# ZikangXiong/mobrob

Hardware: AMD Instinct MI355X
Metric: env-steps/sec (whole node), doggo PPO (higher is better)
Workload: dtype f32

## Files before the change

include/mobrob_ppo.h:

```cpp
#ifndef MOBROB_PPO_H
#define MOBROB_PPO_H

#include <stddef.h>
#include <stdint.h>

#ifdef __cplusplus
extern "C" {
#endif

#define MOBROB_PPO_ABI_VERSION 3
enum { MOBROB_ACT_TANH = 0, MOBROB_ACT_RELU = 1, MOBROB_ACT_ELU = 2, MOBROB_ACT_LEAKY_RELU = 3, MOBROB_ACT_SIGMOID = 4,
       MOBROB_ACT_SOFTPLUS = 5, MOBROB_ACT_SOFTSIGN = 6, MOBROB_ACT_HARDTANH = 7, MOBROB_ACT_RELU6 = 8, MOBROB_ACT_SILU = 9,
       MOBROB_ACT_GELU = 10, MOBROB_ACT_MISH = 11, MOBROB_ACT_COUNT = 12 };

enum {
  MOBROB_OK = 0,
  MOBROB_ERR_INVALID = -1,
  MOBROB_ERR_HIP = -2,
  MOBROB_ERR_STATE = -3,
  MOBROB_ERR_NO_DEVICE = -4
};

typedef struct mobrob_ppo_engine mobrob_ppo_engine_t;

// ... 439 lines not shown
  MOBROB_BUF_RETURNS = 7,
  MOBROB_BUF_PARAMS = 8,
  MOBROB_BUF_GRADS = 9,
  MOBROB_BUF_ADVSTAT = 10,
  MOBROB_BUF_LAST_VALUES = 11,
  MOBROB_BUF_LAST_DONES = 12,
  MOBROB_BUF_CLIPPED_ACTIONS = 13,
  MOBROB_BUF_EPISODE_START_STATE = 14,
  MOBROB_BUF_TERMINAL_OBS = 15,
  MOBROB_BUF_TERMINAL_VALUES = 16,
  MOBROB_BUF_TRUNCATED = 17,
  MOBROB_BUF_ENV_STATE = 18,
  MOBROB_BUF_GRAD_EXCHANGE = 19,
  MOBROB_BUF_SDE_NOISE = 20,
  MOBROB_BUF_COUNT = 21
};
int mobrob_ppo_buffer_info(mobrob_ppo_engine_t* e, int32_t which, void** ptr_dev, size_t* bytes);
int mobrob_ppo_read_buffer(mobrob_ppo_engine_t* e, int32_t which, void* host_out, size_t bytes);
int mobrob_ppo_write_buffer(mobrob_ppo_engine_t* e, int32_t which, const void* host_in, size_t bytes);
int mobrob_ppo_mark_rollout_ready(mobrob_ppo_engine_t* e);

int mobrob_ppo_x3_mode(const mobrob_ppo_engine_t* e);
int mobrob_ppo_update_mode(const mobrob_ppo_engine_t* e);

int mobrob_ppo_explained_variance(mobrob_ppo_engine_t* e, double* out);

int mobrob_ppo_compute_gae(mobrob_ppo_engine_t* e);

int mobrob_ppo_feistel_permutation(mobrob_ppo_engine_t* e, int64_t n, uint64_t key, int64_t* out);

enum {
  MOBROB_K_ACT = 0,
  MOBROB_K_GAE = 1,
  MOBROB_K_TRAIN_GRAD = 2,
  MOBROB_K_APPLY = 3,
  MOBROB_K_ENV = 4,
  MOBROB_K_GRAD_REDUCE = 5,
  MOBROB_K_ALLREDUCE = 6,
  MOBROB_K_COUNT = 7
};
int mobrob_ppo_profile_enable(mobrob_ppo_engine_t* e, int32_t on);
int mobrob_ppo_profile_read(mobrob_ppo_engine_t* e, double* ms , int64_t* calls );

#ifdef __cplusplus
}
#endif
// ... 2 lines not shown
```

mobrob_amd/_lib.py:

```python
from __future__ import annotations

import ctypes as C
import os

_HERE = os.path.dirname(os.path.abspath(__file__))
LIB_PATH = os.environ.get("MOBROB_PPO_LIB") or os.path.join(_HERE, "libmobrob_ppo.so")
ABI_VERSION = 3

OK, ERR_INVALID, ERR_HIP, ERR_STATE, ERR_NO_DEVICE = 0, -1, -2, -3, -4

BUF = dict(obs=0, actions=1, rewards=2, episode_starts=3, values=4, log_probs=5, advantages=6, returns=7,
           params=8, grads=9, advstat=10, last_values=11, last_dones=12, clipped_actions=13, episode_start_state=14,
           terminal_obs=15, terminal_values=16, truncated=17, env_state=18, grad_exchange=19, sde_noise=20)
HYPER = dict(learning_rate=0, clip_range=1, clip_range_vf=2, target_kl=3, ent_coef=4, vf_coef=5, epoch_kernel=6)
KERNEL_IDS = dict(act=0, gae=1, train_grad=2, apply=3, env=4, grad_reduce=5, allreduce=6)


class Config(C.Structure):
    _fields_ = [
        ("abi_version", C.c_int32), ("obs_dim", C.c_int32), ("act_dim", C.c_int32),
        ("pi_hidden", C.c_int32 * 2), ("vf_hidden", C.c_int32 * 2),
        ("n_envs", C.c_int32), ("n_steps", C.c_int32), ("batch_size", C.c_int32), ("n_epochs", C.c_int32),
        ("gamma", C.c_double), ("gae_lambda", C.c_double), ("clip_range", C.c_double), ("ent_coef", C.c_double),
        ("vf_coef", C.c_double), ("max_grad_norm", C.c_double), ("learning_rate", C.c_double),
# ... 202 lines not shown
                                                   C.POINTER(C.c_int32), C.POINTER(C.c_int32), C.POINTER(C.c_int32), C.POINTER(C.c_int32),
                                                   C.POINTER(C.c_int32), C.POINTER(C.c_int32), C.POINTER(C.c_uint16), C.c_int32, _U8,
                                                   C.POINTER(C.c_int32), C.POINTER(C.c_int32), C.POINTER(C.c_int32), C.POINTER(C.c_int32),
                                                   C.POINTER(C.c_int32), C.POINTER(C.c_int32)]),
    "mobrob_ppo_plan_grid_team_smooth": (C.c_int, [_P, C.POINTER(PlanSpec), C.POINTER(WallsC), C.POINTER(HazardFramesC), C.POINTER(PlanTime),
                                                   C.c_int32, C.c_int32, C.c_int32, C.c_int32, _F, _F, _F, C.POINTER(C.c_int32),
                                                   C.POINTER(C.c_int32), C.POINTER(C.c_int32), C.POINTER(C.c_int32), C.POINTER(C.c_int32),
                                                   C.POINTER(C.c_int32), C.POINTER(C.c_int32), C.POINTER(C.c_int32), C.POINTER(C.c_int32),
                                                   C.POINTER(C.c_uint16), C.c_int32, C.POINTER(C.c_int32), C.c_int32, _U8,
                                                   C.POINTER(C.c_int32), C.POINTER(C.c_int32)]),
    "mobrob_ppo_plan_assign": (C.c_int, [_P, C.POINTER(PlanSpec), C.POINTER(WallsC), C.POINTER(HazardsC), C.POINTER(HazardFramesC),
                                         C.POINTER(PlanTime), C.c_int32, C.c_int32, _F, _F, C.POINTER(C.c_int32), _F, C.POINTER(C.c_int32),
                                         _I64, C.POINTER(C.c_int32), _I64, _I64, C.POINTER(C.c_int32), C.POINTER(C.c_int32)]),
    "mobrob_ppo_sde_reset_noise": (C.c_int, [_P]),
    "mobrob_ppo_sde_set_noise": (C.c_int, [_P, _F]),
    "mobrob_ppo_buffer_info": (C.c_int, [_P, C.c_int32, C.POINTER(_P), C.POINTER(C.c_size_t)]),
    "mobrob_ppo_read_buffer": (C.c_int, [_P, C.c_int32, _P, C.c_size_t]),
    "mobrob_ppo_write_buffer": (C.c_int, [_P, C.c_int32, _P, C.c_size_t]),
    "mobrob_ppo_mark_rollout_ready": (C.c_int, [_P]),
    "mobrob_ppo_compute_gae": (C.c_int, [_P]),
    "mobrob_ppo_explained_variance": (C.c_int, [_P, C.POINTER(C.c_double)]),
    "mobrob_ppo_x3_mode": (C.c_int, [_P]),
    "mobrob_ppo_update_mode": (C.c_int, [_P]),
    "mobrob_ppo_feistel_permutation": (C.c_int, [_P, C.c_int64, C.c_uint64, _I64]),
    "mobrob_ppo_profile_enable": (C.c_int, [_P, C.c_int32]),
    "mobrob_ppo_profile_read": (C.c_int, [_P, C.POINTER(C.c_double), _I64]),
}

ALLREDUCE_FN = C.CFUNCTYPE(C.c_int, C.c_void_p, C.c_void_p, C.c_size_t, C.c_int32, C.c_void_p)

_lib = None


class EngineError(RuntimeError):
    pass


def load():
    global _lib
    if _lib is not None:
        return _lib
    if not os.path.exists(LIB_PATH):
        raise ImportError(f"{LIB_PATH} not built. Run `python -c 'import __graft_entry__ as g; g.build()'` "
                          "(hipcc --offload-arch=gfx950). mobrob_amd has no CPU fallback.")
    lib = C.CDLL(LIB_PATH)
    for name, (res, args) in SYMBOLS.items():
# ... 16 lines not shown
```

mobrob_amd/csrc/engine.hip:

```cpp
#include <hip/hip_runtime.h>
#include <rccl/rccl.h>
#include <dlfcn.h>

#include <algorithm>
#include <atomic>
#include <thread>
#include <cmath>
#include <cstdarg>
#include <cstdio>
#include <climits>
#include <cstring>
#include <ctime>
#include <cstdlib>
#include <string>
#include <vector>

#ifdef MOBROB_POISON_LDS
namespace mobrob {
__global__ __launch_bounds__(1024) void k_poison_lds() {
  extern __shared__ unsigned poison_words[];
  volatile unsigned* w = poison_words;
  for (int i = threadIdx.x; i < 160 * 256; i += 1024) w[i] = 0xFFFFFFFFu;
}
inline void poison_lds(hipStream_t st) {
// ... 149 lines not shown
  unsigned adv_pass = 0;
  bool epoch_open = false;
  float* stats = nullptr;
  int stats_cap = 0, stats_n = 0;
  int cur_count = 0;
  bool grad_pending = false;
  double clip_vf = -1.0;
  double target_kl = -1.0;
  int last_epochs_started = 0, last_stopped_early = 0, last_steps_applied = 0;
  ncclComm_t comm = nullptr;
  int64_t allreduce_calls = 0, allreduce_bytes = 0;
  struct OneShot {
    char* xbuf = nullptr;
    size_t payload = 0;
    char* peer[kOneShotMaxRanks] = {nullptr};
    int world = 0, rank = -1;
    bool ready = false;
    unsigned long long seq = 0;
    int* error = nullptr;
    long long timeout_ticks = 0;
  } oneshot;
  double* norm_rec_sum = nullptr; int* norm_rec_t = nullptr; int* fold_idx_dev = nullptr;
  int fold_start[kMaxTensors + 1] = {0};
  bool use_norm_records = false;
  bool epoch_kernel_on = true;
  unsigned* epoch_bar = nullptr;
  float* epoch_consts = nullptr;
  int* epoch_idx = nullptr;
  char* epoch_stage = nullptr;
  int* epoch_err_host = nullptr;
  hipEvent_t epoch_ev = nullptr;
  int last_update_mode = 0;
  float* epoch_snap = nullptr;
  int rollout64_tile_max = 256;
  int pair64_min_tiles = 65;
  int split64_max_tiles = 64;
  float *Xg = nullptr, *actg = nullptr, *lpg = nullptr, *advg = nullptr, *retg = nullptr, *oldvg = nullptr;
  float *hp[kMaxHidden] = {nullptr}, *hv[kMaxHidden] = {nullptr}, *mu = nullptr, *vout = nullptr;
  float *dmu = nullptr, *dv = nullptr, *dzp[kMaxHidden] = {nullptr}, *dzv[kMaxHidden] = {nullptr};
  float *pred_obs = nullptr, *pred_act = nullptr;
  int gemm_tiles = 0;
  bool sde = false, sde_hold = false;
  float *sde_E = nullptr, *sde_E1 = nullptr, *sde_lat2 = nullptr, *sde_gsig = nullptr, *sde_graw = nullptr;
  float *sde_S2 = nullptr, *sde_var = nullptr;
  SdeMode sde_mode{1, 0};
  hipStream_t cstream = nullptr;
  hipEvent_t ev_in = nullptr, ev_k = nullptr, ev_store = nullptr;
// ... 403 lines not shown
}
FusedTrainArgs train256_args(const mobrob_ppo_engine* e) {
  const FusedState& f = e->fused;
  FusedTrainArgs a{};
  a.net[0] = f.net[0]; a.net[1] = f.net[1];
  a.obs = e->obs; a.Dp = e->Dp; a.A = e->A; a.rec = f.train_rec; a.RW = train_rec_width(e->A);
  fill_loss_hyper(e, a);
  a.slabs = f.slabs; a.slab_floats = f.slab_floats; a.sums = e->grads + e->P; a.stamps = f.stamps;
  return a;
}
template <class Args>
Args reduce_args(const mobrob_ppo_engine* e) {
  Args s{};
  s.slabs = e->fused.slabs; s.grads = e->grads; s.P = e->P;
  for (int i = 0; i < 14; ++i) s.offs[i] = e->offs[i];
  s.D = e->D; s.A = e->A; s.ent_coef = (float)e->cfg.ent_coef; s.sums = e->grads + e->P;
  s.rec_sum = e->use_norm_records ? e->norm_rec_sum : nullptr; s.rec_t = e->norm_rec_t;
  return s;
}
Slab64ReduceArgs slab64_reduce_args(const mobrob_ppo_engine* e) { return reduce_args<Slab64ReduceArgs>(e); }
SlabReduceArgs slab_reduce_args(const mobrob_ppo_engine* e) {
  SlabReduceArgs s = reduce_args<SlabReduceArgs>(e);
  s.slab_floats = e->fused.slab_floats; s.Dp = e->Dp; s.h16 = e->A <= 16;
  return s;
}
StatsArgs stats_args(const mobrob_ppo_engine* e) {
  StatsArgs st{};
  st.loss_sums = e->grads + e->P; st.log_std = e->params + e->offs[T_LOGSTD]; st.n_act = e->A; st.sde = e->sde;
  st.ent_coef = (float)e->cfg.ent_coef; st.vf_coef = (float)e->cfg.vf_coef;
  return st;
}
int fused_carve_packs(mobrob_ppo_engine* e) {
  FusedState& f = e->fused;
  const int H = f.H;
  const size_t nW1 = (size_t)(H / 32) * (e->Dp / 8) * 256, nW2 = (size_t)(H / 32) * (H / 8) * 256;
  const size_t nW3f = (size_t)(H / 8) * 256, nW3b = (size_t)(H / 32) * 4 * 256;
  const size_t nW3h = (size_t)(H / 16) * 256;
  const size_t per_net = nW1 + 2 * nW2 + nW3f + nW3h + nW3b + 2 * H;
  f.packed_floats = 2 * per_net;
  CHK(dalloc(e, &f.packed, f.packed_floats));
  const int head_bias[2] = {T_AB, T_VB};
  for (int n = 0; n < 2; ++n) {
    float* p = f.packed + n * per_net;
    f.net[n].W1f = reinterpret_cast<const f32x4*>(p); p += nW1;
    f.net[n].W2f = reinterpret_cast<const f32x4*>(p); p += nW2;
    f.net[n].W3f = reinterpret_cast<const f32x4*>(p); p += nW3f;
// ... 43 lines not shown
          unsigned* w1 = nullptr; unsigned* w2 = nullptr; unsigned* w2b = nullptr; float* w3 = nullptr; float* w3b = nullptr;
          CHK(dalloc(e, &w1, (size_t)K1 * 16 * 768));
          CHK(dalloc(e, &w2, (size_t)8 * 16 * 768));
          CHK(dalloc(e, &w2b, (size_t)8 * 16 * 768));
          CHK(dalloc(e, &w3, (size_t)16 * 64 * 4));
          CHK(dalloc(e, &w3b, (size_t)16 * 64 * 4));
          f.net[n].W1c = w1; f.net[n].W2c = w2; f.net[n].W2bc = w2b; f.net[n].W3c = w3; f.net[n].W3bc = w3b;
        }
        f.lds_chain_bytes = chain_lds_bytes(e->Dp);
      }
    }
    CHK(dalloc(e, &f.train_rec, (size_t)e->N * e->T * train_rec_width(e->A)));
    f.lds_bytes = fused_lds_bytes(e->Dp);
    f.lds_act_bytes = fused_lds_act_bytes(e->Dp);
  }
  return dalloc(e, &f.stamps, 32);
}
int build_norm_record_tables(mobrob_ppo_engine* e) {
  const FusedState& f = e->fused;
  const int nb = cdiv(f.slab_floats, 256);
  CHK(dalloc(e, &e->norm_rec_sum, (size_t)2 * nb * kNormRec));
  CHK(dalloc(e, &e->norm_rec_t, (size_t)2 * nb * kNormRec));
  CHK(dalloc(e, &e->fold_idx_dev, (size_t)2 * nb * kNormRec));
  const SlabReduceArgs s256 = slab_reduce_args(e);
  const Slab64ReduceArgs s64 = slab64_reduce_args(e);
  std::vector<std::vector<int>> per_tensor(13);
  for (int net = 0; net < 2; ++net)
    for (int b = 0; b < nb; ++b) {
      std::vector<int> recs;
      for (int w = 0; w < 4; ++w) {
        std::vector<int> wave;
        for (int l = 0; l < 64; ++l) {
          const int p = b * 256 + w * 64 + l;
          const int dst = p < f.slab_floats ? (f.H == 64 ? slab64_to_canonical(s64, net, p) : slab_to_canonical(s256, net, p)) : -1;
          const int t = tensor_of_canonical(e->offs, e->P, dst);
          if (t >= 0 && std::find(wave.begin(), wave.end(), t) == wave.end()) wave.push_back(t);
        }
        for (int t : wave)
          if (recs.empty() || recs.back() != t) recs.push_back(t);
      }
      if ((int)recs.size() > kNormRec) return fail(MOBROB_ERR_INVALID, "norm record table: %zu tensors in one reduction block", recs.size());
      for (size_t k = 0; k < recs.size(); ++k) per_tensor[recs[k]].push_back((net * nb + b) * kNormRec + (int)k);
    }
  std::vector<int> fold;
  for (int t = 0; t < 13; ++t) {
    e->fold_start[t] = (int)fold.size();
    fold.insert(fold.end(), per_tensor[t].begin(), per_tensor[t].end());
  }
  e->fold_start[13] = (int)fold.size();
  if (fold.size() > 1024) return fail(MOBROB_ERR_INVALID, "norm record table too large (%zu)", fold.size());
  if (!e->plan_only)
    HIPC(hipMemcpyAsync(e->fold_idx_dev, fold.data(), fold.size() * sizeof(int), hipMemcpyHostToDevice, e->stream));
  if (!e->plan_only) HIPC(hipStreamSynchronize(e->stream));
  return MOBROB_OK;
}

int fused_init(mobrob_ppo_engine* e) {
  FusedState& f = e->fused;
  f.enabled = e->cfg.fast_kernels && e->cfg.activation == MOBROB_ACT_TANH && e->Lp == 2 && e->Lv == 2 && !e->sde &&
              fused_shape_ok(e->D, e->A, e->H1, e->H2, e->G1, e->G2);
  if (!f.enabled) return MOBROB_OK;
  f.D = e->D; f.Dp = e->Dp; f.A = e->A; f.H = e->H1;
  if ((uint64_t)(e->T + 1) * e->N * e->Dp * 4ull >= (1ull << 32) || (uint64_t)e->T * e->N * e->A * 4ull >= (1ull << 32) ||
      (uint64_t)e->T * e->N * train_rec_width(e->A) * 4ull >= (1ull << 32)) {
    f.enabled = false;
    return MOBROB_OK;
  }
  CHK(fused_carve_packs(e));
  CHK(fused_alloc_buffers(e));
  if (!e->plan_only) HIPC(fused_set_lds_attr(f));
  return build_norm_record_tables(e);
}
// ... 390 lines not shown
  HIPC(hipMemcpyAsync(e->chunks_dev, e->chunk_table.data(), e->chunk_table.size() * sizeof(NormChunk), hipMemcpyHostToDevice, e->stream));
  std::vector<float> ones(e->N, 1.0f);
  HIPC(hipMemcpyAsync(e->prev_dones, ones.data(), (size_t)e->N * 4, hipMemcpyHostToDevice, e->stream));
  HIPC(hipStreamSynchronize(e->stream));
  repack(e);
  if (e->sde) sde_resample(e, 0, e->N, e->draw_counter++, nullptr, true);
  HIPC(hipStreamSynchronize(e->stream));
  return MOBROB_OK;
}

}

extern "C" {

int mobrob_ppo_device_bytes(const mobrob_ppo_config_t* cfg, size_t* bytes) {
  if (!cfg || !bytes) return fail(MOBROB_ERR_INVALID, "null argument");
  CHK(check_cfg(cfg));
  mobrob_ppo_engine plan;
  plan.plan_only = true;
  CHK(engine_dims(&plan, cfg));
  CHK(engine_alloc(&plan));
  *bytes = plan.arena_used;
  return MOBROB_OK;
}

void* mobrob_ppo_device_alloc(int32_t device_id, size_t bytes) {
  void* p = nullptr;
  if (hipSetDevice(device_id) != hipSuccess || hipMalloc(&p, bytes) != hipSuccess) {
    fail(MOBROB_ERR_HIP, "device_alloc(%zu bytes) failed", bytes);
    return nullptr;
  }
  return p;
}
void mobrob_ppo_device_free(void* p) { if (p) (void)hipFree(p); }

int mobrob_ppo_create(const mobrob_ppo_config_t* cfg, mobrob_ppo_engine_t** out) {
  if (!cfg || !out) return fail(MOBROB_ERR_INVALID, "null argument");
  return engine_create(cfg, nullptr, 0, out);
}

int mobrob_ppo_create_in_arena(const mobrob_ppo_config_t* cfg, void* arena, size_t arena_bytes, mobrob_ppo_engine_t** out) {
  if (!cfg || !out || !arena) return fail(MOBROB_ERR_INVALID, "null argument");
  return engine_create(cfg, arena, arena_bytes, out);
}

void mobrob_ppo_destroy(mobrob_ppo_engine_t* e) {
// ... 1024 lines not shown

int mobrob_ppo_minibatch_grad(mobrob_ppo_engine_t* e, int32_t mb) {
  if (!e) return fail(MOBROB_ERR_INVALID, "null engine");
  if (!e->epoch_open) return fail(MOBROB_ERR_STATE, "minibatch_grad before epoch_begin");
  if (mb < 0 || mb >= e->nmb) return fail(MOBROB_ERR_INVALID, "minibatch %d out of range [0,%d)", mb, e->nmb);
  const int start = mb * e->Bl, B = std::min(e->Bl, e->N * e->T - start);
  const float inv_bg = 1.0f / (float)((int64_t)B * e->cfg.world_size);
  e->cur_count = B;
  if (!e->fused.enabled) generic_minibatch_grad(e, mb, start, B, inv_bg);
  else if (e->fused.H == 64) fused64_minibatch_grad(e, mb, start, B, inv_bg);
  else fused_minibatch_grad(e, mb, start, B, inv_bg);
  HIPC(hipGetLastError());
  e->grad_pending = true;
  return MOBROB_OK;
}

namespace {
void fill_adam_pack_args(mobrob_ppo_engine* e, AdamPackArgs& a) {
  a.p = e->params; a.g = e->grads; a.m = e->m; a.v = e->v; a.P = e->P;
  a.chunks = e->chunks_dev; a.partial = e->chunk_partial; a.nchunks = e->nchunks;
  if (e->use_norm_records) {
    a.partial = e->norm_rec_sum; a.fold_idx = e->fold_idx_dev;
    for (int i = 0; i <= kMaxTensors; ++i) a.fold_start[i] = e->fold_start[i];
  }
  a.max_norm = (float)e->cfg.max_grad_norm; a.beta1 = (float)e->cfg.adam_beta1; a.beta2 = (float)e->cfg.adam_beta2;
  a.eps = (float)e->cfg.adam_eps;
  for (int i = 0; i <= kMaxTensors; ++i) a.offs[i] = e->offs[i];
  a.ntens = e->ntens; a.two_by_two = e->Lp == 2 && e->Lv == 2; a.id_pw1 = T_PW1; a.id_vw1 = T_VW1; a.id_aw = T_AW; a.id_vw = T_VW; a.HL = e->HL; a.GL = e->GL;
  a.D = e->D; a.Dp = e->Dp; a.A = e->A; a.Ap = e->Ap; a.H1 = e->H1; a.H2 = e->H2; a.G1 = e->G1; a.G2 = e->G2;
  a.pW1p = e->pW1p; a.vW1p = e->vW1p; a.aWp = e->aWp; a.vWp = e->vWp;
  for (int n = 0; n < 2; ++n) {
    const bool on = e->fused.enabled;
    a.fW1f[n] = on ? (float*)e->fused.net[n].W1f : nullptr;
    a.fW2f[n] = on ? (float*)e->fused.net[n].W2f : nullptr;
    a.fW3f[n] = on ? (float*)e->fused.net[n].W3f : nullptr;
    const bool ch = on && e->fused.train_chain;
    a.fW2b[n] = on && !ch ? (float*)e->fused.net[n].W2b : nullptr;
    a.fW3b[n] = on && !ch ? (float*)e->fused.net[n].W3b : nullptr;
    a.fW3h[n] = (on && (n == 1 || e->fused.A <= 16)) ? (float*)e->fused.net[n].W3h : nullptr;
    a.fb1s[n] = on ? (float*)e->fused.net[n].b1s : nullptr;
    a.fb2s[n] = on ? (float*)e->fused.net[n].b2s : nullptr;
    const bool x3 = on && e->fused.train_x3;
    a.xW1[n] = x3 ? reinterpret_cast<unsigned short*>(const_cast<unsigned*>(e->fused.net[n].W1x)) : nullptr;
    a.xW2[n] = x3 ? reinterpret_cast<unsigned short*>(const_cast<unsigned*>(e->fused.net[n].W2x)) : nullptr;
    a.xW2b[n] = x3 && !ch ? reinterpret_cast<unsigned short*>(const_cast<unsigned*>(e->fused.net[n].W2bx)) : nullptr;
    a.cW1[n] = ch ? reinterpret_cast<unsigned short*>(const_cast<unsigned*>(e->fused.net[n].W1c)) : nullptr;
    a.cW2[n] = ch ? reinterpret_cast<unsigned short*>(const_cast<unsigned*>(e->fused.net[n].W2c)) : nullptr;
// ... 12 lines not shown
  return {(float)(e->cfg.learning_rate / bc1), (float)std::sqrt(bc2)};
}
int next_stats_row(mobrob_ppo_engine* e) {
  if (e->stats_n >= e->stats_cap) e->stats_n = 0;
  return e->stats_n++;
}
StatsArgs apply_norms(mobrob_ppo_engine* e) {
  StatsArgs st = stats_args(e);
  st.stats_row = e->stats + (size_t)next_stats_row(e) * 8;
  st.inv_bg = 1.0f / (float)((int64_t)e->cur_count * e->cfg.world_size);
  if (!e->use_norm_records)
    hipLaunchKernelGGL(k_sqnorm_chunks, dim3(e->nchunks), dim3(256), 0, e->stream, e->grads, e->chunks_dev,
                       e->chunk_partial, st);
  return st;
}
int apply_adam(mobrob_ppo_engine* e, const StatsArgs& st) {
  const AdamStep step = next_adam_step(e);
  AdamPackArgs a{};
  fill_adam_pack_args(e, a);
  a.step_size = step.step_size; a.bc2_sqrt = step.bc2_sqrt;
  if (e->use_norm_records) a.st = st;
  a.stats_row = st.stats_row;
  a.loss_sums_zero = e->fused.enabled ? e->grads + e->P : nullptr;
  hipLaunchKernelGGL(k_adam_pack, dim3(cdiv(e->P, 256)), dim3(256), 0, e->stream, a);
  HIPC(hipGetLastError());
  e->grad_pending = false;
  return MOBROB_OK;
}
}

namespace {
int apply_checked(mobrob_ppo_engine* e, int32_t* stopped) {
  *stopped = 0;
  ProfScope ps(e, MOBROB_K_APPLY);
  const StatsArgs st = apply_norms(e);
  if (e->target_kl > 0.0) {
    float approx_kl = 0.f;
    HIPC(hipMemcpyAsync(&approx_kl, st.stats_row + 4, sizeof(float), hipMemcpyDeviceToHost, e->stream));
    HIPC(hipStreamSynchronize(e->stream));
    if ((double)approx_kl > 1.5 * e->target_kl) {
      *stopped = 1;
      e->grad_pending = false;
      HIPC(hipMemsetAsync(st.stats_row + 6, 0xFF, sizeof(float), e->stream));
      if (e->fused.enabled) HIPC(hipMemsetAsync(e->grads + e->P, 0, 8 * sizeof(float), e->stream));
      return MOBROB_OK;
    }
  }
// ... 239 lines not shown
      if (le == hipSuccess) le = hipLaunchCooperativeKernel(fn, dim3(launch.grid), dim3(256), kargs, (unsigned)kEpochLdsBytes, e->stream);
    }));
    if (le != hipSuccess) return fail(MOBROB_ERR_HIP, "k_epoch64 launch (%d workgroups): %s", launch.grid, hipGetErrorString(le));
  }
  e->cur_count = std::min(e->Bl, total - (nmb - 1) * e->Bl);
  e->grad_pending = false;
  e->last_steps_applied += nmb;
  return MOBROB_OK;
}

int train_loop(mobrob_ppo_engine* e, const int64_t* perms, bool dp, bool records, mobrob_allreduce_fn fn, void* ctx) {
  if (!dp && e->cfg.world_size != 1)
    return fail(MOBROB_ERR_STATE, "mobrob_ppo_train is the single-rank loop; data-parallel ranks call mobrob_ppo_train_dp "
                                  "(or drive epoch_begin/minibatch_grad/[all-reduce]/minibatch_apply)");
  const size_t total = (size_t)e->N * e->T;
  e->stats_n = 0;
  const bool kl = e->target_kl > 0.0;
  e->last_epochs_started = 0; e->last_stopped_early = 0; e->last_steps_applied = 0;
  struct RecordsOn {
    mobrob_ppo_engine* e;
    RecordsOn(mobrob_ppo_engine* e_, bool on) : e(e_) { e->use_norm_records = on; }
    ~RecordsOn() { e->use_norm_records = false; }
  } records_on(e, records);
  EpochLaunch epoch_launch;
  const bool epoch_kernel = epoch_kernel_eligible(e, dp, records, &epoch_launch);
  e->last_update_mode = epoch_kernel ? 1 : 0;
  for (int ep = 0; ep < e->cfg.n_epochs; ++ep) {
    CHK(mobrob_ppo_epoch_begin(e, perms ? perms + (size_t)ep * total : nullptr));
    if (dp) CHK(dp_all_reduce(e, e->advstat, (size_t)e->nmb * 4, 1, fn, ctx));
    e->last_epochs_started = ep + 1;
    if (ep == e->cfg.n_epochs - 1 || kl) e->stats_n = 0;
    if (epoch_kernel) {
      CHK(launch_epoch_kernel(e, ep, epoch_launch));
      continue;
    }
    for (int mb = 0; mb < e->nmb && !e->last_stopped_early; ++mb) {
      CHK(mobrob_ppo_minibatch_grad(e, mb));
      if (dp) CHK(dp_all_reduce(e, e->grads, (size_t)e->P + 8, 0, fn, ctx));
      int32_t stopped = 0;
      CHK(apply_checked(e, &stopped));
      if (stopped) {
        e->last_stopped_early = 1;
        break;
      }
      e->last_steps_applied++;
    }
    if (e->last_stopped_early) break;
  }
  e->epoch_open = false;
// ... 2280 lines not shown
```

mobrob_amd/csrc/kernels_fused.h:

```cpp
#pragma once
#include "device_utils.h"

namespace mobrob {

constexpr int FH = 256;
constexpr int FR = 64;
constexpr int FLDH = FH + 4;
constexpr int FLDO = 36;
constexpr int FTHREADS = 256;

struct FusedNet {
  const f32x4* W1f;
  const f32x4* W2f;
  const f32x4* W3f;
  const f32x4* W3h;
  const f32x4* W2b;
  const f32x4* W3b;
  const float* b1s; const float* b2s;
  const float* b3;
  int head;
  const unsigned* W1x;
  const unsigned* W2x;
  const unsigned* W2bx;
  const unsigned* W1c;
// ... 1407 lines not shown
  {
    const float t0 = wave_sum(s_pl), t1 = wave_sum(s_vl), t2 = wave_sum(s_kl), t3 = wave_sum(s_cf);
    if (lane == 0) {
      lds[L::STAT + wave * 4 + 0] = t0;
      lds[L::STAT + wave * 4 + 1] = t1;
      lds[L::STAT + wave * 4 + 2] = t2;
      lds[L::STAT + wave * 4 + 3] = t3;
    }
    __syncthreads();
    if (tid < 4)
      slab[slab_off_st(DP) + tid] = (lds[L::STAT + tid] + lds[L::STAT + 4 + tid]) + (lds[L::STAT + 8 + tid] + lds[L::STAT + 12 + tid]);
  }
}

struct SlabReduceArgs {
  const float* slabs; int slab_floats; int nslabs;
  float* grads; int P;
  int offs[14];
  int D, Dp, A;
  int h16;
  float ent_coef, b_local, inv_bg;
  float* sums;
  double* rec_sum; int* rec_t;
};

constexpr int kNormRec = 4;
template <class PI>
__host__ __device__ inline int tensor_of_canonical(PI offs, int P, int dst) {
  if (dst < 0 || dst >= P) return -1;
  int t = 0;
  for (int k = 1; k < 13; ++k) t += (dst >= offs[k]) ? 1 : 0;
  return t;
}
template <bool COH = false>
__device__ __forceinline__ void block_norm_records(int t, float val, double* rec_sum, int* rec_t) {
  __shared__ double sc[4 * kNormRec];
  __shared__ int sct[4 * kNormRec];
  const int lane = threadIdx.x & 63, wave = threadIdx.x >> 6;
  const double sq = t >= 0 ? (double)val * (double)val : 0.0;
  int nrec = 0;
  unsigned long long todo = __ballot(t >= 0);
  while (todo != 0ull) {
    const int first = __ffsll((long long)todo) - 1;
    const int tsel = __shfl(t, first, 64);
    const bool m = t == tsel;
    const double sum = wave_sum_d(m ? sq : 0.0);
    if (lane == 0 && nrec < kNormRec) { sc[wave * kNormRec + nrec] = sum; sct[wave * kNormRec + nrec] = tsel; }
    ++nrec;
    todo &= ~__ballot(m);
  }
  if (lane == 0)
    for (int k = nrec; k < kNormRec; ++k) sct[wave * kNormRec + k] = -1;
  __syncthreads();
  if (threadIdx.x == 0) {
    int n = 0, cur = -1;
    double acc = 0.0;
    for (int k = 0; k < 4 * kNormRec; ++k) {
      const int tt = sct[k];
      if (tt < 0) continue;
      if (tt == cur) { acc += sc[k]; continue; }
      if (cur >= 0 && n < kNormRec) { stc<COH>(rec_sum + n, acc); stc<COH>(rec_t + n, cur); ++n; }
      cur = tt;
      acc = sc[k];
    }
    if (cur >= 0 && n < kNormRec) { stc<COH>(rec_sum + n, acc); stc<COH>(rec_t + n, cur); ++n; }
    for (; n < kNormRec; ++n) stc<COH>(rec_t + n, -1);
  }
}

__host__ __device__ __forceinline__ int slab_to_canonical(const SlabReduceArgs& s, int net, int p) {
  const int T_W1 = net == 0 ? 1 : 5, T_B1 = net == 0 ? 2 : 6, T_W2 = net == 0 ? 3 : 7, T_B2 = net == 0 ? 4 : 8;
  const int T_W3 = net == 0 ? 9 : 11, T_B3 = net == 0 ? 10 : 12;
  const int head = net == 0 ? s.A : 1;
  auto frag = [](int q, int nt, int* w, int* t, int* i, int* lane) {
    *lane = (q >> 2) & 63;
    *i = (q & 3) + 4 * ((q >> 8) & 3);
    const int wt = q >> 10;
    *t = wt % nt;
    *w = wt / nt;
  };
  int w, t, i, lane;
  if (p < slab_off_w1()) {
    frag(p, 16, &w, &t, &i, &lane);
    const int n = 64 * w + 32 * (t >> 3) + crc(i) + 4 * (lane >> 5), j = 32 * (t & 7) + (lane & 31);
    return s.offs[T_W2] + n * FH + j;
  }
  if (p < slab_off_w3(s.Dp)) {
    frag(p - slab_off_w1(), 4, &w, &t, &i, &lane);
    const int n = 64 * w + 32 * (t >> 1) + crc(i) + 4 * (lane >> 5), j = 32 * (t & 1) + (lane & 31);
    return j < s.D ? s.offs[T_W1] + n * s.D + j : -1;
  }
// ... 43 lines not shown
#pragma unroll
    for (int k = 0; k < U; ++k) ac[k] = 0.f;
    int w = 0;
    for (; w + U <= n; w += U) {
      float v[U];
#pragma unroll
      for (int k = 0; k < U; ++k) v[k] = src[(size_t)(w + k) * stride];
#pragma unroll
      for (int k = 0; k < U; ++k) ac[k] += v[k];
    }
#pragma unroll
    for (int k = 0; k < U; ++k)
      if (w + k < n) ac[k] += src[(size_t)(w + k) * stride];
#pragma unroll
    for (int d = U / 2; d >= 1; d >>= 1)
#pragma unroll
      for (int k = 0; k < d; ++k) ac[k] += ac[k + d];
    acc = ac[0];
    if (dst < s.offs[1]) acc = __fadd_rn(acc, __fmul_rn(__fmul_rn(s.ent_coef, -s.b_local), s.inv_bg));
    s.grads[dst] = acc;
  }
  if (s.rec_sum != nullptr) {
    const size_t b = ((size_t)net * gridDim.x + blockIdx.x) * kNormRec;
    block_norm_records(tensor_of_canonical(s.offs, s.P, dst), acc, s.rec_sum + b, s.rec_t + b);
  }
}

__global__ void k_pack_fwd(const float* __restrict__ W, int N, int K, int ld, float* __restrict__ out, int NB,
                           int KG, float scale) {
  const int i = blockIdx.x * blockDim.x + threadIdx.x;
  if (i >= NB * KG * 256) return;
  const int s = i & 3, lane = (i >> 2) & 63, kg = (i >> 8) % KG, nb = (i >> 8) / KG;
  const int n = nb * 32 + (lane & 31), k = kg * 8 + 4 * (lane >> 5) + s;
  out[i] = (n < N && k < K) ? scale * W[(size_t)n * ld + k] : 0.f;
}
__host__ __device__ inline int pack_h16_idx(int n, int k) { return (((k >> 4) * 64) + 16 * ((k >> 2) & 3) + n) * 4 + (k & 3); }
__global__ void k_pack_h16(const float* __restrict__ W, int N, int K, float* __restrict__ out) {
  const int i = blockIdx.x * blockDim.x + threadIdx.x;
  if (i >= (K / 16) * 256) return;
  const int s = i & 3, lane = (i >> 2) & 63, kg = i >> 8;
  const int n = lane & 15, k = 16 * kg + 4 * (lane >> 4) + s;
  out[i] = n < N ? W[(size_t)n * K + k] : 0.f;
}
__global__ void k_scale_copy(const float* __restrict__ src, float* __restrict__ dst, int n, float scale) {
  const int i = blockIdx.x * blockDim.x + threadIdx.x;
  if (i < n) dst[i] = scale * src[i];
}
// ... 261 lines not shown
}

constexpr int kMaxTensors = 1 + 4 * kMaxHidden + 4;
constexpr int kFusedTensors = 17;
struct AdamPackArgs {
  float* p; const float* g; float* m; float* v; int P;
  float* g_out;
  const NormChunk* chunks; const double* partial; int nchunks;
  const int* fold_idx; int fold_start[kMaxTensors + 1];
  float max_norm, step_size, bc2_sqrt, beta1, beta2, eps;
  int offs[kMaxTensors + 1];
  int ntens;
  int two_by_two;
  int id_pw1, id_vw1, id_aw, id_vw;
  int HL, GL;
  int D, Dp, A, Ap, H1, H2, G1, G2;
  float* pW1p; float* vW1p; float* aWp; float* vWp;
  float* fW1f[2]; float* fW2f[2]; float* fW3f[2]; float* fW3h[2]; float* fW2b[2]; float* fW3b[2]; float* fb1s[2]; float* fb2s[2];
  unsigned short* xW1[2]; unsigned short* xW2[2]; unsigned short* xW2b[2];
  unsigned short* cW1[2]; unsigned short* cW2[2]; unsigned short* cW2b[2]; float* cW3[2]; float* cW3b[2];
  float* stats_row;
  float* loss_sums_zero;
  StatsArgs st;
};

__device__ __forceinline__ int pack_fwd_idx(int n, int k, int KG) {
  return (((n >> 5) * KG + (k >> 3)) * 64 + (n & 31) + 32 * ((k >> 2) & 1)) * 4 + (k & 3);
}
__device__ __forceinline__ int pack_bwd_idx(int krow, int j, int KG) {
  return (((j >> 5) * KG + (krow >> 3)) * 64 + (j & 31) + 32 * ((krow >> 2) & 1)) * 4 + (krow & 3);
}

__device__ __forceinline__ void x3_pack_store(unsigned short* out, int n, int k, int KS, float x) {
  asm volatile("" : "+v"(x));
  unsigned p1, p2, p3;
  x3_split2(x, 0.f, p1, p2, p3);
  const size_t base = ((size_t)((n >> 5) * KS + (k >> 4)) * 3) * 512 + (size_t)((n & 31) + 32 * ((k & 15) >> 3)) * 8 + (k & 7);
  out[base] = (unsigned short)(p1 & 0xffffu);
  out[base + 512] = (unsigned short)(p2 & 0xffffu);
  out[base + 1024] = (unsigned short)(p3 & 0xffffu);
}
__host__ __device__ __forceinline__ void chain_kslot_of_neuron(int n, int* s, int* g, int* j) {
  *s = n >> 5;
  const int r = n & 31;
  *g = (r >> 2) & 3;
  *j = ((r >> 4) << 2) | (r & 3);
// ... 34 lines not shown
  const float pn = __fmaf_rn(-step_size, __fdiv_rn(m, denom), p0);
  int t = 0;
#pragma unroll
  for (int k = 1; k < kFusedTensors; ++k) t += (i >= a.offs[k]) ? 1 : 0;
  if (a.ntens > kFusedTensors)
    for (int k = kFusedTensors; k < a.ntens; ++k) t += (i >= a.offs[k]) ? 1 : 0;
  const int e = i - a.offs[t];
  a.m[i] = m;
  a.v[i] = v;
  if (COH && a.two_by_two && (t == 0 || t == 10 || t == 12)) stc<true>(a.p + i, pn);
  else a.p[i] = pn;
#ifdef ADAM_NO_PACK
  return;
#endif
  if (!a.two_by_two) {
    if (t == a.id_pw1 || t == a.id_vw1) {
      const int n = e / a.D, k = e - n * a.D;
      (t == a.id_vw1 ? a.vW1p : a.pW1p)[n * a.Dp + k] = pn;
    } else if (t == a.id_aw || t == a.id_vw) {
      (t == a.id_vw ? a.vWp : a.aWp)[e] = pn;
    }
    return;
  }
  switch (t) {
    case 1: case 5: {
      const int net = t == 5, n = e / a.D, k = e - n * a.D;
      (net ? a.vW1p : a.pW1p)[n * a.Dp + k] = pn;
      if (a.fW1f[net]) stc<COH>(a.fW1f[net] + pack_fwd_idx(n, k, a.Dp / 8), kTanhScale * pn);
      if (a.xW1[net]) x3_pack_store(a.xW1[net], n, k, a.Dp / 16, kTanhScale * pn);
      if (a.cW1[net]) chain_store_w1(a.cW1[net], n, k, (a.Dp + 31) / 32, kTanhScale * pn);
    } break;
    case 3: case 7: {
      const int net = t == 7;
      if (a.fW2f[net]) {
        const int K = net ? a.G1 : a.H1, n = e / K, k = e - n * K;
        stc<COH>(a.fW2f[net] + pack_fwd_idx(n, k, K / 8), kTanhScale * pn);
        if (a.fW2b[net]) stc<COH>(a.fW2b[net] + pack_bwd_idx(n, k, (net ? a.G2 : a.H2) / 8), pn);
        if (a.xW2[net]) x3_pack_store(a.xW2[net], n, k, K / 16, kTanhScale * pn);
        if (a.xW2b[net]) x3_pack_store(a.xW2b[net], k, n, (net ? a.G2 : a.H2) / 16, pn);
        if (a.cW2[net]) chain_store_w2(a.cW2[net], a.cW2b[net], n, k, kTanhScale * pn, pn);
      }
    } break;
    case 9: case 11: {
      const int net = t == 11, K = net ? a.G2 : a.H2, n = e / K, k = e - n * K;
      (net ? a.vWp : a.aWp)[e] = pn;
      if (a.fW3f[net]) {
        stc<COH>(a.fW3f[net] + pack_fwd_idx(n, k, K / 8), pn);
        if (a.fW3b[net]) stc<COH>(a.fW3b[net] + pack_bwd_idx(n, k, 4), pn);
        if (a.fW3h[net] && n < 16) stc<COH>(a.fW3h[net] + pack_h16_idx(n, k), pn);
        if (a.cW3[net] && n < 16) { a.cW3[net][chain_head_fwd_idx(n, k)] = pn; a.cW3b[net][chain_head_bwd_idx(n, k)] = pn; }
      }
    } break;
    case 2: case 6: if (a.fb1s[t == 6]) stc<COH>(a.fb1s[t == 6] + e, kTanhScale * pn); break;
    case 4: case 8: if (a.fb2s[t == 8]) stc<COH>(a.fb2s[t == 8] + e, kTanhScale * pn); break;
    default: break;
  }
}

template <bool COH, class TA>
__device__ __forceinline__ void adam_pack_block_at(const TA& a, int lin, int i, float g_in, float m_in, float v_in, float p_in, float step_size,
                                                   float bc2_sqrt, float* stats_row, float inv_bg, float ent_pre, int fidx_pre = -1) {
  __shared__ double part[1024];
  __shared__ int tens[256];
  __shared__ float nts[kMaxTensors + 3];
  __shared__ float coef_s, total_s;
  if (lin == 0 && a.st.loss_sums != nullptr) {
    StatsArgs st;
    st.stats_row = stats_row; st.loss_sums = a.st.loss_sums; st.log_std = a.st.log_std;
    st.ent_coef = a.st.ent_coef; st.vf_coef = a.st.vf_coef; st.inv_bg = inv_bg; st.n_act = a.st.n_act; st.sde = a.st.sde;
    stats_row_from_sums<COH>(st, ent_pre);
  }
  if (a.fold_idx != nullptr) {
    const int nrec = a.fold_start[13];
    if (nrec <= 128) {
      if ((int)threadIdx.x < nrec) part[threadIdx.x] = ldc<COH>(a.partial + (fidx_pre >= 0 ? fidx_pre : a.fold_idx[threadIdx.x]));
      __syncthreads();
      if (threadIdx.x < 13) {
        double ts = 0.0;
        for (int c = a.fold_start[threadIdx.x]; c < a.fold_start[threadIdx.x + 1]; ++c) ts += part[c];
        nts[threadIdx.x] = (float)sqrt(ts);
      }
    } else {
      const int lane = threadIdx.x & 63, wv = threadIdx.x >> 6;
      const bool staged = nrec <= 1024;
      if (staged) {
        for (int c = threadIdx.x; c < nrec; c += blockDim.x) part[c] = ldc<COH>(a.partial + a.fold_idx[c]);
        __syncthreads();
      }
      for (int t = wv; t < 13; t += 4) {
        double ts = 0.0;
        if (staged)
          for (int c = a.fold_start[t] + lane; c < a.fold_start[t + 1]; c += 64) ts += part[c];
        else
          for (int c = a.fold_start[t] + lane; c < a.fold_start[t + 1]; c += 64) ts += ldc<COH>(a.partial + a.fold_idx[c]);
        ts = wave_sum_d(ts);
        if (lane == 0) nts[t] = (float)sqrt(ts);
      }
    }
  } else {
    for (int c = threadIdx.x; c < a.nchunks; c += blockDim.x) {
      part[c] = ldc<COH>(a.partial + c);
      tens[c] = a.chunks[c].tensor;
    }
    __syncthreads();
    if ((int)threadIdx.x < a.ntens) {
      double ts = 0.0;
      for (int c = 0; c < a.nchunks; ++c)
        if (tens[c] == (int)threadIdx.x) ts += part[c];
      nts[threadIdx.x] = (float)sqrt(ts);
    }
  }
  __syncthreads();
  if (threadIdx.x == 0) {
    float tot_sq = 0.f;
    for (int t = 0; t < a.ntens; ++t) tot_sq = __fmaf_rn(nts[t], nts[t], tot_sq);
    const float total = sqrtf(tot_sq);
    total_s = total;
    coef_s = fminf(a.max_norm / (total + 1e-6f), 1.0f);
  }
  __syncthreads();
  const float coef = coef_s;
  if (lin == 0 && stats_row != nullptr) stats_row[6] = total_s;
  if (lin < 8 && a.loss_sums_zero != nullptr) stc<COH>(a.loss_sums_zero + lin, 0.f);
  if (i < 0 || i >= a.P) return;
  adam_pack_apply<COH>(a, i, g_in, m_in, v_in, p_in, coef, step_size, bc2_sqrt);
}
template <bool COH, class TA>
__device__ __forceinline__ void adam_pack_block(const TA& a, int bx, float step_size, float bc2_sqrt, float* stats_row, float inv_bg) {
  const int i = bx * 256 + (int)threadIdx.x;
  float g_in = 0.f, m_in = 0.f, v_in = 0.f, p_in = 0.f;
  if (i < a.P) { g_in = ldc<COH>(a.g + i); m_in = ldc<COH>(a.m + i); v_in = ldc<COH>(a.v + i); p_in = ldc<COH>(a.p + i); }
  const float ent = (i == 0 && a.st.loss_sums != nullptr) ? entropy_of_log_std<COH>(a.st.log_std, a.st.n_act) : 0.f;
  adam_pack_block_at<COH>(a, i, i, g_in, m_in, v_in, p_in, step_size, bc2_sqrt, stats_row, inv_bg, ent);
}
__global__ __launch_bounds__(256) void k_adam_pack(AdamPackArgs a) {
  adam_pack_block<false>(a, blockIdx.x, a.step_size, a.bc2_sqrt, a.stats_row, a.st.inv_bg);
}

struct FusedState {
  bool enabled = false;
  int H = 0;
  int D = 0, Dp = 0, A = 0;
  float* packed = nullptr;
  size_t packed_floats = 0;
  FusedNet net[2];
  float* slabs = nullptr;
  float* train_rec = nullptr;
  bool train_x3 = false;
  bool train_chain = false;
  size_t lds_chain_bytes = 0;
  unsigned long long* stamps = nullptr;
  int slab_floats = 0, max_grid = 0;
  int pair_nseq_max = 0;
  size_t lds_bytes = 0, lds_act_bytes = 0;
};

inline size_t fused_lds_bytes(int Dp) { return (size_t)(FR * (Dp + 4) + 2 * FR * FLDH + FR * FLDO + 96 + 256 + 16) * sizeof(float); }

inline size_t fused_lds_act_bytes(int Dp) { return (size_t)(32 * (Dp + 4) + 2 * 32 * FLDH + 4 * 32 * FLDO) * sizeof(float); }
// ... 47 lines not shown
```

Baseline: 32.75 million.

## Fold grad-norm records once in last reducer block, pack only chain weights in tail

After: 32.79 million (median of 6 runs). No clear change (+0.1%).

```diff
diff --git a/include/mobrob_ppo.h b/include/mobrob_ppo.h
--- a/include/mobrob_ppo.h
+++ b/include/mobrob_ppo.h
@@ -485,6 +485,7 @@
 
 int mobrob_ppo_x3_mode(const mobrob_ppo_engine_t* e);
 int mobrob_ppo_update_mode(const mobrob_ppo_engine_t* e);
+int mobrob_ppo_norm_fold_table(const mobrob_ppo_config_t* cfg, int32_t* fold_start14, int32_t* fold_idx, int32_t cap);
 
 int mobrob_ppo_explained_variance(mobrob_ppo_engine_t* e, double* out);
 
diff --git a/mobrob_amd/_lib.py b/mobrob_amd/_lib.py
--- a/mobrob_amd/_lib.py
+++ b/mobrob_amd/_lib.py
@@ -248,6 +248,7 @@
     "mobrob_ppo_explained_variance": (C.c_int, [_P, C.POINTER(C.c_double)]),
     "mobrob_ppo_x3_mode": (C.c_int, [_P]),
     "mobrob_ppo_update_mode": (C.c_int, [_P]),
+    "mobrob_ppo_norm_fold_table": (C.c_int, [C.POINTER(Config), C.POINTER(C.c_int32), C.POINTER(C.c_int32), C.c_int32]),
     "mobrob_ppo_feistel_permutation": (C.c_int, [_P, C.c_int64, C.c_uint64, _I64]),
     "mobrob_ppo_profile_enable": (C.c_int, [_P, C.c_int32]),
     "mobrob_ppo_profile_read": (C.c_int, [_P, C.POINTER(C.c_double), _I64]),
diff --git a/mobrob_amd/csrc/engine.hip b/mobrob_amd/csrc/engine.hip
--- a/mobrob_amd/csrc/engine.hip
+++ b/mobrob_amd/csrc/engine.hip
@@ -195,7 +195,11 @@
   } oneshot;
   double* norm_rec_sum = nullptr; int* norm_rec_t = nullptr; int* fold_idx_dev = nullptr;
   int fold_start[kMaxTensors + 1] = {0};
+  std::vector<int> fold_host;
   bool use_norm_records = false;
+  float* norm_out = nullptr; unsigned* norm_ticket = nullptr;
+  bool fold_once = false;
+  bool pack_chain_only = false;
   bool epoch_kernel_on = true;
   unsigned* epoch_bar = nullptr;
   float* epoch_consts = nullptr;
@@ -645,6 +649,10 @@
 SlabReduceArgs slab_reduce_args(const mobrob_ppo_engine* e) {
   SlabReduceArgs s = reduce_args<SlabReduceArgs>(e);
   s.slab_floats = e->fused.slab_floats; s.Dp = e->Dp; s.h16 = e->A <= 16;
+  if (e->fold_once && s.rec_sum != nullptr) {
+    s.ticket = e->norm_ticket; s.fold_idx = e->fold_idx_dev; s.norm_out = e->norm_out;
+    for (int i = 0; i < 14; ++i) s.fold_start[i] = e->fold_start[i];
+  }
   return s;
 }
 StatsArgs stats_args(const mobrob_ppo_engine* e) {
@@ -734,6 +742,8 @@
   CHK(dalloc(e, &e->norm_rec_sum, (size_t)2 * nb * kNormRec));
   CHK(dalloc(e, &e->norm_rec_t, (size_t)2 * nb * kNormRec));
   CHK(dalloc(e, &e->fold_idx_dev, (size_t)2 * nb * kNormRec));
+  CHK(dalloc(e, &e->norm_out, 16));
+  CHK(dalloc(e, &e->norm_ticket, 1));
   const SlabReduceArgs s256 = slab_reduce_args(e);
   const Slab64ReduceArgs s64 = slab64_reduce_args(e);
   std::vector<std::vector<int>> per_tensor(13);
@@ -760,6 +770,7 @@
     fold.insert(fold.end(), per_tensor[t].begin(), per_tensor[t].end());
   }
   e->fold_start[13] = (int)fold.size();
+  e->fold_host = fold;
   if (fold.size() > 1024) return fail(MOBROB_ERR_INVALID, "norm record table too large (%zu)", fold.size());
   if (!e->plan_only)
     HIPC(hipMemcpyAsync(e->fold_idx_dev, fold.data(), fold.size() * sizeof(int), hipMemcpyHostToDevice, e->stream));
@@ -1196,6 +1207,20 @@
   CHK(engine_alloc(&plan));
   *bytes = plan.arena_used;
   return MOBROB_OK;
+}
+
+int mobrob_ppo_norm_fold_table(const mobrob_ppo_config_t* cfg, int32_t* fold_start14, int32_t* fold_idx, int32_t cap) {
+  if (!cfg || !fold_start14 || !fold_idx) return fail(MOBROB_ERR_INVALID, "null argument");
+  CHK(check_cfg(cfg));
+  mobrob_ppo_engine plan;
+  plan.plan_only = true;
+  CHK(engine_dims(&plan, cfg));
+  CHK(engine_alloc(&plan));
+  if (!plan.fused.enabled) return 0;
+  if ((int)plan.fold_host.size() > cap) return fail(MOBROB_ERR_INVALID, "norm_fold_table: %zu entries, room for %d", plan.fold_host.size(), cap);
+  for (int t = 0; t < 14; ++t) fold_start14[t] = plan.fold_start[t];
+  for (size_t k = 0; k < plan.fold_host.size(); ++k) fold_idx[k] = plan.fold_host[k];
+  return (int)plan.fold_host.size();
 }
 
 void* mobrob_ppo_device_alloc(int32_t device_id, size_t bytes) {
@@ -2266,7 +2291,9 @@
   if (e->use_norm_records) {
     a.partial = e->norm_rec_sum; a.fold_idx = e->fold_idx_dev;
     for (int i = 0; i <= kMaxTensors; ++i) a.fold_start[i] = e->fold_start[i];
-  }
+    if (e->fold_once) { a.norm_in = e->norm_out; a.ticket_zero = e->norm_ticket; }
+  }
+  a.chain_only = e->pack_chain_only ? 1 : 0;
   a.max_norm = (float)e->cfg.max_grad_norm; a.beta1 = (float)e->cfg.adam_beta1; a.beta2 = (float)e->cfg.adam_beta2;
   a.eps = (float)e->cfg.adam_eps;
   for (int i = 0; i <= kMaxTensors; ++i) a.offs[i] = e->offs[i];
@@ -2325,7 +2352,8 @@
   if (e->use_norm_records) a.st = st;
   a.stats_row = st.stats_row;
   a.loss_sums_zero = e->fused.enabled ? e->grads + e->P : nullptr;
-  hipLaunchKernelGGL(k_adam_pack, dim3(cdiv(e->P, 256)), dim3(256), 0, e->stream, a);
+  if (a.norm_in != nullptr) hipLaunchKernelGGL(k_adam_pack_folded, dim3(cdiv(e->P, 256)), dim3(256), 0, e->stream, a);
+  else hipLaunchKernelGGL(k_adam_pack, dim3(cdiv(e->P, 256)), dim3(256), 0, e->stream, a);
   HIPC(hipGetLastError());
   e->grad_pending = false;
   return MOBROB_OK;
@@ -2611,9 +2639,19 @@
     RecordsOn(mobrob_ppo_engine* e_, bool on) : e(e_) { e->use_norm_records = on; }
     ~RecordsOn() { e->use_norm_records = false; }
   } records_on(e, records);
+  const bool short_tail = !dp && e->fused.enabled && e->fused.H == FH && e->fused.train_chain && !env_switched_off("MOBROB_TAIL_V1");
+  struct ShortTail {
+    mobrob_ppo_engine* e; bool on;
+    ShortTail(mobrob_ppo_engine* e_, bool on_, bool fold) : e(e_), on(on_) { e->pack_chain_only = on; e->fold_once = on && fold; }
+    ~ShortTail() {
+      e->pack_chain_only = false; e->fold_once = false;
+      if (on) repack(e);
+    }
+  } tail(e, short_tail, records && getenv("MOBROB_TAIL_FOLD_ONCE") != nullptr);
+  if (e->fold_once) HIPC(hipMemsetAsync(e->norm_ticket, 0, sizeof(unsigned), e->stream));
   EpochLaunch epoch_launch;
   const bool epoch_kernel = epoch_kernel_eligible(e, dp, records, &epoch_launch);
-  e->last_update_mode = epoch_kernel ? 1 : 0;
+  e->last_update_mode = (epoch_kernel ? 1 : 0) | (e->fold_once ? 2 : 0) | (short_tail ? 4 : 0);
   for (int ep = 0; ep < e->cfg.n_epochs; ++ep) {
     CHK(mobrob_ppo_epoch_begin(e, perms ? perms + (size_t)ep * total : nullptr));
     if (dp) CHK(dp_all_reduce(e, e->advstat, (size_t)e->nmb * 4, 1, fn, ctx));
diff --git a/mobrob_amd/csrc/kernels_fused.h b/mobrob_amd/csrc/kernels_fused.h
--- a/mobrob_amd/csrc/kernels_fused.h
+++ b/mobrob_amd/csrc/kernels_fused.h
@@ -1453,6 +1453,7 @@
   float ent_coef, b_local, inv_bg;
   float* sums;
   double* rec_sum; int* rec_t;
+  unsigned* ticket; const int* fold_idx; int fold_start[14]; float* norm_out;
 };
 
 constexpr int kNormRec = 4;
@@ -1498,6 +1499,30 @@
     for (; n < kNormRec; ++n) stc<COH>(rec_t + n, -1);
   }
 }
+template <bool COH, class TA>
+__device__ __forceinline__ void fold_records_wide(const TA& a, const double* partial, int nrec, double* part, float* nts) {
+  const int lane = threadIdx.x & 63, wv = threadIdx.x >> 6;
+  const bool staged = nrec <= 1024;
+  if (staged) {
+    for (int c = threadIdx.x; c < nrec; c += blockDim.x) part[c] = ldc<COH>(partial + a.fold_idx[c]);
+    __syncthreads();
+  }
+  for (int t = wv; t < 13; t += 4) {
+    double ts = 0.0;
+    if (staged)
+      for (int c = a.fold_start[t] + lane; c < a.fold_start[t + 1]; c += 64) ts += part[c];
+    else
+      for (int c = a.fold_start[t] + lane; c < a.fold_start[t + 1]; c += 64) ts += ldc<COH>(partial + a.fold_idx[c]);
+    ts = wave_sum_d(ts);
+    if (lane == 0) nts[t] = (float)sqrt(ts);
+  }
+}
+__device__ __forceinline__ float total_norm_of(const float* nts, int ntens) {
+  float tot_sq = 0.f;
+  for (int t = 0; t < ntens; ++t) tot_sq = __fmaf_rn(nts[t], nts[t], tot_sq);
+  return sqrtf(tot_sq);
+}
+__device__ __forceinline__ float clip_coef_of(float max_norm, float total) { return fminf(max_norm / (total + 1e-6f), 1.0f); }
 
 __host__ __device__ __forceinline__ int slab_to_canonical(const SlabReduceArgs& s, int net, int p) {
   const int T_W1 = net == 0 ? 1 : 5, T_B1 = net == 0 ? 2 : 6, T_W2 = net == 0 ? 3 : 7, T_B2 = net == 0 ? 4 : 8;
@@ -1587,7 +1612,28 @@
   }
   if (s.rec_sum != nullptr) {
     const size_t b = ((size_t)net * gridDim.x + blockIdx.x) * kNormRec;
-    block_norm_records(tensor_of_canonical(s.offs, s.P, dst), acc, s.rec_sum + b, s.rec_t + b);
+    const int t = tensor_of_canonical(s.offs, s.P, dst);
+    if (s.ticket == nullptr) {
+      block_norm_records(t, acc, s.rec_sum + b, s.rec_t + b);
+      return;
+    }
+    block_norm_records<true>(t, acc, s.rec_sum + b, s.rec_t + b);
+    __shared__ double part[1024];
+    __shared__ float nts[16];
+    __shared__ int last_s;
+    if (threadIdx.x == 0) {
+      asm volatile("s_waitcnt vmcnt(0)" ::: "memory");
+      const unsigned tk = __hip_atomic_fetch_add(s.ticket, 1u, __ATOMIC_RELAXED, __HIP_MEMORY_SCOPE_AGENT);
+      const int last = tk == gridDim.x * gridDim.y - 1u;
+      if (last) __builtin_amdgcn_fence(__ATOMIC_ACQUIRE, "agent");
+      last_s = last;
+    }
+    __syncthreads();
+    if (!last_s) return;
+    fold_records_wide<true>(s, s.rec_sum, s.fold_start[13], part, nts);
+    __syncthreads();
+    if (threadIdx.x < 13) s.norm_out[threadIdx.x] = nts[threadIdx.x];
+    if (threadIdx.x == 0) s.norm_out[13] = total_norm_of(nts, 13);
   }
 }
 
@@ -1895,6 +1941,9 @@
   float* stats_row;
   float* loss_sums_zero;
   StatsArgs st;
+  int chain_only;
+  const float* norm_in;
+  unsigned* ticket_zero;
 };
 
 __device__ __forceinline__ int pack_fwd_idx(int n, int k, int KG) {
@@ -1975,32 +2024,39 @@
     }
     return;
   }
+  const bool all = a.chain_only == 0;
   switch (t) {
     case 1: case 5: {
       const int net = t == 5, n = e / a.D, k = e - n * a.D;
-      (net ? a.vW1p : a.pW1p)[n * a.Dp + k] = pn;
-      if (a.fW1f[net]) stc<COH>(a.fW1f[net] + pack_fwd_idx(n, k, a.Dp / 8), kTanhScale * pn);
-      if (a.xW1[net]) x3_pack_store(a.xW1[net], n, k, a.Dp / 16, kTanhScale * pn);
+      if (all) {
+        (net ? a.vW1p : a.pW1p)[n * a.Dp + k] = pn;
+        if (a.fW1f[net]) stc<COH>(a.fW1f[net] + pack_fwd_idx(n, k, a.Dp / 8), kTanhScale * pn);
+        if (a.xW1[net]) x3_pack_store(a.xW1[net], n, k, a.Dp / 16, kTanhScale * pn);
+      }
       if (a.cW1[net]) chain_store_w1(a.cW1[net], n, k, (a.Dp + 31) / 32, kTanhScale * pn);
     } break;
     case 3: case 7: {
       const int net = t == 7;
       if (a.fW2f[net]) {
         const int K = net ? a.G1 : a.H1, n = e / K, k = e - n * K;
-        stc<COH>(a.fW2f[net] + pack_fwd_idx(n, k, K / 8), kTanhScale * pn);
-        if (a.fW2b[net]) stc<COH>(a.fW2b[net] + pack_bwd_idx(n, k, (net ? a.G2 : a.H2) / 8), pn);
-        if (a.xW2[net]) x3_pack_store(a.xW2[net], n, k, K / 16, kTanhScale * pn);
-        if (a.xW2b[net]) x3_pack_store(a.xW2b[net], k, n, (net ? a.G2 : a.H2) / 16, pn);
+        if (all) {
+          stc<COH>(a.fW2f[net] + pack_fwd_idx(n, k, K / 8), kTanhScale * pn);
+          if (a.fW2b[net]) stc<COH>(a.fW2b[net] + pack_bwd_idx(n, k, (net ? a.G2 : a.H2) / 8), pn);
+          if (a.xW2[net]) x3_pack_store(a.xW2[net], n, k, K / 16, kTanhScale * pn);
+          if (a.xW2b[net]) x3_pack_store(a.xW2b[net], k, n, (net ? a.G2 : a.H2) / 16, pn);
+        }
         if (a.cW2[net]) chain_store_w2(a.cW2[net], a.cW2b[net], n, k, kTanhScale * pn, pn);
       }
     } break;
     case 9: case 11: {
       const int net = t == 11, K = net ? a.G2 : a.H2, n = e / K, k = e - n * K;
-      (net ? a.vWp : a.aWp)[e] = pn;
+      if (all) (net ? a.vWp : a.aWp)[e] = pn;
       if (a.fW3f[net]) {
-        stc<COH>(a.fW3f[net] + pack_fwd_idx(n, k, K / 8), pn);
-        if (a.fW3b[net]) stc<COH>(a.fW3b[net] + pack_bwd_idx(n, k, 4), pn);
-        if (a.fW3h[net] && n < 16) stc<COH>(a.fW3h[net] + pack_h16_idx(n, k), pn);
+        if (all) {
+          stc<COH>(a.fW3f[net] + pack_fwd_idx(n, k, K / 8), pn);
+          if (a.fW3b[net]) stc<COH>(a.fW3b[net] + pack_bwd_idx(n, k, 4), pn);
+          if (a.fW3h[net] && n < 16) stc<COH>(a.fW3h[net] + pack_h16_idx(n, k), pn);
+        }
         if (a.cW3[net] && n < 16) { a.cW3[net][chain_head_fwd_idx(n, k)] = pn; a.cW3b[net][chain_head_bwd_idx(n, k)] = pn; }
       }
     } break;
@@ -2034,21 +2090,7 @@
         nts[threadIdx.x] = (float)sqrt(ts);
       }
     } else {
-      const int lane = threadIdx.x & 63, wv = threadIdx.x >> 6;
-      const bool staged = nrec <= 1024;
-      if (staged) {
-        for (int c = threadIdx.x; c < nrec; c += blockDim.x) part[c] = ldc<COH>(a.partial + a.fold_idx[c]);
-        __syncthreads();
-      }
-      for (int t = wv; t < 13; t += 4) {
-        double ts = 0.0;
-        if (staged)
-          for (int c = a.fold_start[t] + lane; c < a.fold_start[t + 1]; c += 64) ts += part[c];
-        else
-          for (int c = a.fold_start[t] + lane; c < a.fold_start[t + 1]; c += 64) ts += ldc<COH>(a.partial + a.fold_idx[c]);
-        ts = wave_sum_d(ts);
-        if (lane == 0) nts[t] = (float)sqrt(ts);
-      }
+      fold_records_wide<COH>(a, a.partial, nrec, part, nts);
     }
   } else {
     for (int c = threadIdx.x; c < a.nchunks; c += blockDim.x) {
@@ -2065,11 +2107,9 @@
   }
   __syncthreads();
   if (threadIdx.x == 0) {
-    float tot_sq = 0.f;
-    for (int t = 0; t < a.ntens; ++t) tot_sq = __fmaf_rn(nts[t], nts[t], tot_sq);
-    const float total = sqrtf(tot_sq);
+    const float total = total_norm_of(nts, a.ntens);
     total_s = total;
-    coef_s = fminf(a.max_norm / (total + 1e-6f), 1.0f);
+    coef_s = clip_coef_of(a.max_norm, total);
   }
   __syncthreads();
   const float coef = coef_s;
@@ -2088,6 +2128,22 @@
 }
 __global__ __launch_bounds__(256) void k_adam_pack(AdamPackArgs a) {
   adam_pack_block<false>(a, blockIdx.x, a.step_size, a.bc2_sqrt, a.stats_row, a.st.inv_bg);
+}
+__global__ __launch_bounds__(256) void k_adam_pack_folded(AdamPackArgs a) {
+  const int i = blockIdx.x * 256 + (int)threadIdx.x;
+  float g_in = 0.f, m_in = 0.f, v_in = 0.f, p_in = 0.f;
+  if (i < a.P) { g_in = a.g[i]; m_in = a.m[i]; v_in = a.v[i]; p_in = a.p[i]; }
+  __builtin_amdgcn_sched_barrier(0);
+  const float total = a.norm_in[13];
+  if (blockIdx.x == 0) {
+    if (i == 0 && a.st.loss_sums != nullptr) stats_row_from_sums(a.st, entropy_of_log_std(a.st.log_std, a.st.n_act));
+    __syncthreads();
+    if (i == 0 && a.stats_row != nullptr) a.stats_row[6] = total;
+    if (i < 8 && a.loss_sums_zero != nullptr) a.loss_sums_zero[i] = 0.f;
+    if (i == 8) *a.ticket_zero = 0u;
+  }
+  if (i >= a.P) return;
+  adam_pack_apply(a, i, g_in, m_in, v_in, p_in, clip_coef_of(a.max_norm, total), a.step_size, a.bc2_sqrt);
 }
 
 struct FusedState {
```
